# geoeo/ORB_SLAM3_V1.0

Hardware: AMD Instinct MI355X
Metric: frames/sec ORB extract+match, 752x480 8-level 1000-feat; bit-exact kp/desc (higher is better)
Workload: dtype u8

## Files before the change

### orb_slam3_v1.0_amd/csrc/fast_common.h

```cpp
#pragma once
#include <hip/hip_runtime.h>
#include <stdint.h>

namespace orbfe {

constexpr int kFastTW = 64, kFastTH = 32;

__device__ __forceinline__ bool arc9(uint32_t m)
{
    uint32_t m2 = m | (m << 16);
    uint32_t r = m2 & (m2 >> 1);
    r &= r >> 2;
    r &= r >> 4;
    r &= m2 >> 8;
    return (r & 0xffffu) != 0;
}

__device__ __forceinline__ bool corner_at_global(const uint8_t* __restrict__ img, int pitch, int x, int y, int th)
{
    const int8_t dy[16] = {3, 3, 2, 1, 0, -1, -2, -3, -3, -3, -2, -1, 0, 1, 2, 3};
    const int8_t dx[16] = {0, 1, 2, 3, 3, 3, 2, 1, 0, -1, -2, -3, -3, -3, -2, -1};
    const int v = img[(size_t)y * pitch + x];
    uint32_t mb = 0, md = 0;
#pragma unroll
    for (int k = 0; k < 16; k++) {
        const int d = (int)img[(size_t)(y + dy[k]) * pitch + x + dx[k]] - v;
        mb |= (uint32_t)(d > th) << k;
        md |= (uint32_t)(d < -th) << k;
    }
    return arc9(mb) || arc9(md);
}

}
```

### orb_slam3_v1.0_amd/csrc/kernels_fast.hip

```cpp
#include <cstdlib>

#include "launch.h"
#include "device_math.h"
#include "fast_common.h"

namespace orbfe {

constexpr int kImgW = kFastTW + 8, kImgH = kFastTH + 8;
constexpr int kScH = kFastTH + 2;
constexpr int kScW = kFastTW + 2;
constexpr int kScPitch = kImgW;
constexpr int kScoreOfs = 3 * kImgW + 3;
constexpr int kMaxTileCand = (kFastTW / 2) * (kFastTH / 2);
constexpr int kTmpH = kFastTH + 4;
constexpr int kQCap = 2304;
static_assert(kQCap >= kScH * kScW && kQCap % 2 == 0, "stage A geometry");

typedef unsigned short u16x2 __attribute__((ext_vector_type(2)));


__device__ __forceinline__ unsigned long long mask_le_u32(uint32_t x, uint32_t bound)
{
    unsigned long long m;
    asm("v_cmp_le_u32_e64 %0, %1, %2" : "=s"(m) : "v"(x), "s"(bound));
// ... 32 lines not shown
{
    unsigned long long m;
    if (vbound) asm("v_cmp_lt_i32_e64 %0, %1, %2" : "=s"(m) : "v"(a), "v"(b));
    else asm("v_cmp_lt_i32_e64 %0, %1, %2" : "=s"(m) : "v"(a), "s"(b));
    return m;
}
__device__ __forceinline__ void masked_lds_write_b8(unsigned long long mask, uint32_t addr, uint32_t v)
{
    unsigned long long save;
    asm volatile("s_and_saveexec_b64 %0, %1\n\tds_write_b8 %2, %3\n\ts_mov_b64 exec, %0" : "=&s"(save) : "s"(mask), "v"(addr), "v"(v) : "scc", "memory");
}
__device__ __forceinline__ void masked_lds_write_b16(unsigned long long mask, uint32_t addr, uint32_t v)
{
    unsigned long long save;
    asm volatile("s_and_saveexec_b64 %0, %1\n\tds_write_b16 %2, %3\n\ts_mov_b64 exec, %0" : "=&s"(save) : "s"(mask), "v"(addr), "v"(v) : "scc", "memory");
}
__device__ __forceinline__ void lds_add(uint32_t* addr, uint32_t v)
{
    asm volatile("ds_add_u32 %0, %1" : : "v"((uint32_t)(uintptr_t)addr), "v"(v) : "memory");
}

__device__ __forceinline__ uint32_t lds_add_rtn(uint32_t* addr, uint32_t v)
{
    uint32_t old;
    asm volatile("ds_add_rtn_u32 %0, %1, %2\n\ts_waitcnt lgkmcnt(0)" : "=&v"(old) : "v"((uint32_t)(uintptr_t)addr), "v"(v) : "memory");
    return old;
}

__device__ __forceinline__ uint32_t min16(uint32_t a, uint32_t b)
{
    uint32_t r;
    asm("v_min_u16 %0, %1, %2" : "=v"(r) : "v"(a), "v"(b));
    return r;
}
__device__ __forceinline__ uint32_t max16(uint32_t a, uint32_t b)
{
    uint32_t r;
    asm("v_max_u16 %0, %1, %2" : "=v"(r) : "v"(a), "v"(b));
    return r;
}
__device__ __forceinline__ uint32_t sub16(uint32_t a, uint32_t b)
{
    uint32_t r;
    asm("v_sub_u16 %0, %1, %2" : "=v"(r) : "v"(a), "v"(b));
    return r;
}
__device__ __forceinline__ uint32_t maxi16(uint32_t a, uint32_t b)
{
    uint32_t r;
    asm("v_max_i16 %0, %1, %2" : "=v"(r) : "v"(a), "v"(b));
    return r;
}

__device__ __forceinline__ uint32_t arc_max_of_min(const uint32_t (&p)[16])
{
    uint32_t S[16], Pf[16];
    S[7] = p[7];
    S[15] = p[15];
#pragma unroll
    for (int k = 6; k >= 0; k--) {
        S[k] = min16(p[k], S[k + 1]);
        S[k + 8] = min16(p[k + 8], S[k + 9]);
    }
    Pf[0] = p[0];
    Pf[8] = p[8];
#pragma unroll
    for (int k = 1; k < 7; k++) {
        Pf[k] = min16(p[k], Pf[k - 1]);
        Pf[k + 8] = min16(p[k + 8], Pf[k + 7]);
    }
    Pf[7] = S[0];
    Pf[15] = S[8];
    uint32_t a[16];
#pragma unroll
    for (int k = 0; k < 8; k++) {
        a[k] = min16(S[k], Pf[k + 8]);
        a[k + 8] = min16(S[k + 8], Pf[k]);
    }
#pragma unroll
    for (int st = 8; st >= 1; st >>= 1)
#pragma unroll
        for (int k = 0; k < st; k++) a[k] = max16(a[k], a[k + st]);
    return a[0];
}

__device__ __forceinline__ uint32_t arc_min_of_max(const uint32_t (&p)[16])
{
    uint32_t S[16], Pf[16];
    S[7] = p[7];
    S[15] = p[15];
#pragma unroll
    for (int k = 6; k >= 0; k--) {
        S[k] = max16(p[k], S[k + 1]);
        S[k + 8] = max16(p[k + 8], S[k + 9]);
    }
    Pf[0] = p[0];
    Pf[8] = p[8];
#pragma unroll
    for (int k = 1; k < 7; k++) {
        Pf[k] = max16(p[k], Pf[k - 1]);
        Pf[k + 8] = max16(p[k + 8], Pf[k + 7]);
    }
    Pf[7] = S[0];
    Pf[15] = S[8];
    uint32_t a[16];
#pragma unroll
    for (int k = 0; k < 8; k++) {
        a[k] = max16(S[k], Pf[k + 8]);
        a[k + 8] = max16(S[k + 8], Pf[k]);
    }
#pragma unroll
    for (int st = 8; st >= 1; st >>= 1)
#pragma unroll
        for (int k = 0; k < st; k++) a[k] = min16(a[k], a[k + st]);
    return a[0];
}

__device__ __forceinline__ unsigned long long mask_th_i16(int th, uint32_t m)
{
    unsigned long long r;
    asm("v_cmp_lt_i16_e64 %0, %1, %2" : "=s"(r) : "s"(th), "v"(m));
    return r;
}

__device__ __forceinline__ int queue_slot1(uint32_t m, int th, unsigned long long mask, uint32_t entry, int stepV, int qNext)
{
    unsigned long long save;
    uint32_t tmp;
    int cnt;
    asm volatile("v_cmp_lt_i16_e32 vcc, %8, %3\n\t"
                 "s_and_b64 vcc, vcc, %4\n\t"
                 "s_and_saveexec_b64 %0, vcc\n\t"
                 "v_mbcnt_lo_u32_b32 %1, vcc_lo, 0\n\t"
                 "v_mbcnt_hi_u32_b32 %1, vcc_hi, %1\n\t"
                 "v_mad_i32_i24 %1, %1, %6, %7\n\t"
                 "ds_write_b16 %1, %5\n\t"
                 "s_mov_b64 exec, %0\n\t"
                 "s_bcnt1_i32_b64 %2, vcc"
                 : "=&s"(save), "=&v"(tmp), "=s"(cnt)
                 : "v"(m), "s"(mask), "v"(entry), "v"(stepV), "s"(qNext), "s"(th)
                 : "vcc", "scc", "memory");
    return cnt;
}

template <int MODE>
__global__ __launch_bounds__(256) void fast_blur_kernel(const PipelineDesc* __restrict__ P,
                                                        const uint32_t* __restrict__ tileInfo,
                                                        const uint8_t* __restrict__ gray0, size_t gray0FrameStride,
                                                        int gray0Pitch, int gray0Aligned4,
                                                        uint8_t* __restrict__ ws, uint32_t* __restrict__ cand,
                                                        uint32_t* __restrict__ counters,
                                                        uint16_t* __restrict__ tileRows)
{
    __shared__ uint32_t sRow[kFastTH];
    __shared__ __attribute__((aligned(16))) uint8_t sImg[kImgH + 1][kImgW];
    __shared__ __attribute__((aligned(16))) uint32_t sTmp[kTmpH / 2][kFastTW];
    __shared__ __attribute__((aligned(16))) uint8_t sScore[kScH + 1][kScPitch];
    __shared__ uint32_t sCand[kMaxTileCand];
    __shared__ uint32_t sCnt[4];
    __shared__ uint32_t sBase;
    __shared__ __attribute__((aligned(4))) uint16_t sQA[kQCap];
    static_assert(sizeof(uint16_t) * kScH * kScW <= sizeof(uint32_t) * (kTmpH / 2) * kFastTW, "corner queue must fit the blur buffer");
    uint16_t* const sQB = reinterpret_cast<uint16_t*>(&sTmp[0][0]);
    __shared__ uint32_t sQ[3];

    const int f = blockIdx.x;
    const int tile = blockIdx.y;
    const int nL = P->nLevels;
    const uint32_t ti = tileInfo[tile];
    const int l = (int)(ti >> 24);
    const LevelDesc& L = P->lv[l];
    const int w = L.w, h = L.h;
    const int x0 = (int)(ti & 0xfffu) * kFastTW;
    const int y0 = (int)((ti >> 12) & 0xfffu) * kFastTH;
    const int minTh = P->minTh, iniTh = P->iniTh;

    const uint8_t* src;
    int spitch;
    bool aligned;
    if (l == 0) {
        src = gray0 + (size_t)f * gray0FrameStride;
        spitch = gray0Pitch;
        aligned = gray0Aligned4 != 0;
    } else {
        src = ws + L.imgOff + (size_t)f * L.imgFrameStride;
        spitch = L.pitch;
        aligned = true;
    }

    const int tid = threadIdx.x;
    const int lane = tid & 63;
    if (tid < 4) sCnt[tid] = 0;
    if (tid < 3) sQ[tid] = 0;
    if (tid < kFastTH) sRow[tid] = 0;

    if (aligned) {
        if (tid < 14 * (kImgW / 4)) {
            const int r0 = tid / (kImgW / 4);
            const int c4 = tid - r0 * (kImgW / 4);
            const int gx = x0 - 4 + 4 * c4;
            const bool colIn = gx >= 0 && gx < w;
            uint32_t wv[3];
            if (y0 >= 4 && y0 + kFastTH + 4 <= h) {
                uint32_t off = __umul24((unsigned)(y0 - 4 + r0), (unsigned)spitch) + (unsigned)gx;
                const uint32_t step = 14u * (unsigned)spitch;
#pragma unroll
                for (int k = 0; k < 3; k++) {
                    wv[k] = 0;
                    if (colIn && r0 + 14 * k < kImgH) wv[k] = *reinterpret_cast<const uint32_t*>(src + off);
                    off += step;
                }
            } else {
#pragma unroll
                for (int k = 0; k < 3; k++) {
                    const int r = r0 + 14 * k;
                    wv[k] = 0;
                    if (colIn && r < kImgH)
                        wv[k] = *reinterpret_cast<const uint32_t*>(src + (size_t)reflect_near(y0 - 4 + r, h) * spitch + gx);
                }
            }
#pragma unroll
            for (int k = 0; k < 3; k++) {
                const int r = r0 + 14 * k;
                if (colIn && r < kImgH) *reinterpret_cast<uint32_t*>(&sImg[r][4 * c4]) = wv[k];
            }
        }
        const int cR = w - x0 + 4;
        const bool patchL = x0 == 0, patchR = cR + 1 < kImgW;
        if (patchL || patchR) {
            __syncthreads();
            if (tid < kImgH) {
                if (patchL) {
                    sImg[tid][2] = sImg[tid][6];
                    sImg[tid][3] = sImg[tid][5];
                }
            } else if (tid >= 64 && tid < 64 + kImgH) {
                if (patchR) {
                    sImg[tid - 64][cR] = sImg[tid - 64][cR - 2];
                    sImg[tid - 64][cR + 1] = sImg[tid - 64][cR - 3];
                }
            }
        }
    } else {
        for (int e = tid; e < kImgH * (kImgW / 4); e += 256) {
            const int r = e / (kImgW / 4);
            const int c4 = e - r * (kImgW / 4);
            const uint8_t* row = src + (size_t)reflect_near(y0 - 4 + r, h) * spitch;
            uint32_t wv = 0;
#pragma unroll
            for (int i = 0; i < 4; i++) wv |= (uint32_t)row[reflect_near(x0 - 4 + 4 * c4 + i, w)] << (8 * i);
            *reinterpret_cast<uint32_t*>(&sImg[r][4 * c4]) = wv;
        }
    }
    __syncthreads();

    if constexpr ((MODE & 1) != 0) {
    for (int e = tid; e < (kTmpH / 2) * (kFastTW / 4); e += 256) {
        const int j = e / (kFastTW / 4);
        const int xl = (e - j * (kFastTW / 4)) * 4;
        uint32_t o[2][4];
#pragma unroll
        for (int half = 0; half < 2; half++) {
            const uint32_t* rowp = reinterpret_cast<const uint32_t*>(&sImg[2 * j + half + 2][xl]);
            const uint32_t w0 = rowp[0], w1 = rowp[1], w2 = rowp[2];
            uint32_t win[5];
            win[0] = __builtin_amdgcn_alignbyte(w1, w0, 2);
            win[1] = __builtin_amdgcn_alignbyte(w1, w0, 3);
            win[2] = w1;
            win[3] = __builtin_amdgcn_alignbyte(w2, w1, 1);
            win[4] = __builtin_amdgcn_alignbyte(w2, w1, 2);
#pragma unroll
            for (int i = 0; i < 4; i++)
                o[half][i] = __builtin_amdgcn_udot4(win[i + 1], 0x16000000u,
                                                    __builtin_amdgcn_udot4(win[i], 0x3E583E16u, 0u, false), false);
        }
        uint4 pk;
        pk.x = o[0][0] | (o[1][0] << 16);
        pk.y = o[0][1] | (o[1][1] << 16);
        pk.z = o[0][2] | (o[1][2] << 16);
        pk.w = o[0][3] | (o[1][3] << 16);
        *reinterpret_cast<uint4*>(&sTmp[j][xl]) = pk;
    }
    __syncthreads();
    }

    const int wv = __builtin_amdgcn_readfirstlane(tid >> 6);
    if (wv >= 2) {
        if constexpr ((MODE & 2) != 0)
            for (int e = tid - 128; e < (kScH + 1) * (kScPitch / 4); e += 128) reinterpret_cast<uint32_t*>(&sScore[0][0])[e] = 0;
        if constexpr ((MODE & 1) != 0) {
            uint8_t* dst = ws + L.blurOff + (size_t)f * L.blurFrameStride;
            const int dpitch = L.pitch;
            const int xl = (tid & 15) * 4;
#pragma unroll 1
            for (int yp = (tid - 128) >> 4; yp < kFastTH / 2; yp += 8) {
                const int gy = y0 + 2 * yp, gx = x0 + xl;
                if (gy < h && gx < w) {
                    const uint4 p0 = *reinterpret_cast<const uint4*>(&sTmp[yp][xl]);
                    const uint4 p1 = *reinterpret_cast<const uint4*>(&sTmp[yp + 1][xl]);
                    const uint4 p2 = *reinterpret_cast<const uint4*>(&sTmp[yp + 2][xl]);
                    const uint32_t c0[4] = {p0.x, p0.y, p0.z, p0.w}, c1[4] = {p1.x, p1.y, p1.z, p1.w}, c2[4] = {p2.x, p2.y, p2.z, p2.w};
                    uint32_t ev[4], od[4];
#pragma unroll
                    for (int i = 0; i < 4; i++) {
                        const u16x2 a = __builtin_bit_cast(u16x2, c0[i]), b = __builtin_bit_cast(u16x2, c1[i]), c = __builtin_bit_cast(u16x2, c2[i]);
                        uint32_t acc = __builtin_amdgcn_udot2(a, __builtin_bit_cast(u16x2, 0x003E0016u), 32768u, false);
                        acc = __builtin_amdgcn_udot2(b, __builtin_bit_cast(u16x2, 0x003E0058u), acc, false);
                        ev[i] = __builtin_amdgcn_udot2(c, __builtin_bit_cast(u16x2, 0x00000016u), acc, false);
                        acc = __builtin_amdgcn_udot2(a, __builtin_bit_cast(u16x2, 0x00160000u), 32768u, false);
                        acc = __builtin_amdgcn_udot2(b, __builtin_bit_cast(u16x2, 0x0058003Eu), acc, false);
                        od[i] = __builtin_amdgcn_udot2(c, __builtin_bit_cast(u16x2, 0x0016003Eu), acc, false);
                    }
                    const uint32_t outE = __builtin_amdgcn_perm(ev[1], ev[0], 0x0c0c0602u) |
                                          (__builtin_amdgcn_perm(ev[3], ev[2], 0x0c0c0602u) << 16);
                    const uint32_t outO = __builtin_amdgcn_perm(od[1], od[0], 0x0c0c0602u) |
                                          (__builtin_amdgcn_perm(od[3], od[2], 0x0c0c0602u) << 16);
                    uint8_t* drow = dst + (size_t)gy * dpitch;
                    const bool odd = gy + 1 < h;
                    if (gx + 3 < w) {
                        *reinterpret_cast<uint32_t*>(drow + gx) = outE;
                        if (odd) *reinterpret_cast<uint32_t*>(drow + dpitch + gx) = outO;
                    } else {
                        for (int i = 0; gx + i < w; i++) {
                            drow[gx + i] = (uint8_t)(outE >> (8 * i));
                            if (odd) drow[dpitch + gx + i] = (uint8_t)(outO >> (8 * i));
                        }
                    }
// ... 156 lines not shown
            masked_lds_add(mPre, rowLds + 4u * oy, select_by_mask(mHi, 0x10001u, 1u));
            if (mKeep) {
                uint32_t wbase = 0;
                if (lane == 0) wbase = lds_add_rtn(&sCnt[0], (uint32_t)__popcll(mKeep));
                wbase = __builtin_amdgcn_readfirstlane(wbase);
                const uint32_t rank = __builtin_amdgcn_mbcnt_hi((uint32_t)(mKeep >> 32), __builtin_amdgcn_mbcnt_lo((uint32_t)mKeep, 0u));
                masked_lds_write_b32(mKeep, candLds + 4u * (wbase + rank), pack_cand(x0 + (int)ox, y0 + (int)oy, (int)sc));
            }
        }
        if (lane == 0) {
            if (nPreW) lds_add(&sCnt[2], nPreW);
            if (nPreHiW) lds_add(&sCnt[3], nPreHiW);
            if (nKeepHiW) lds_add(&sCnt[1], nKeepHiW);
        }
        asm volatile("s_waitcnt lgkmcnt(0)" ::: "memory");
    }
    __syncthreads();

    }

    if (tid < kFastTH) {
        const uint32_t v = sRow[tid];
        tileRows[((size_t)f * P->totalTiles + tile) * kFastTH + tid] = (uint16_t)((v & 0xffu) | ((v >> 16) << 8));
    }

    uint32_t* cnt = counters + ((size_t)f * nL + l) * kCntWords;
    const uint32_t nTile = sCnt[0];
    if (tid == 0) {
        uint32_t base = 0;
        if constexpr ((MODE & 256) != 0) base = (uint32_t)tile * 8u;
        else if (nTile) base = atomicAdd(&cnt[kCntCand], nTile);
        if (sCnt[1]) atomicAdd(&cnt[kCntHigh], sCnt[1]);
        if (sCnt[2]) atomicAdd(&cnt[kCntPreLow], sCnt[2]);
        if (sCnt[3]) atomicAdd(&cnt[kCntPreHigh], sCnt[3]);
        sBase = base;
    }
    __syncthreads();
    if (nTile) {
        const uint32_t base = sBase;
        uint32_t* out = cand + L.candOff + (size_t)f * L.candCap;
        for (uint32_t i = tid; i < nTile; i += 256) {
            if (base + i < (uint32_t)L.candCap) out[base + i] = sCand[i];
            else atomicOr(&cnt[kCntStatus], (uint32_t)kFlagCandOverflow);
        }
    }
}

void fast_tiles_for(int w, int h, int* tx, int* ty)
{
    *tx = (w + kFastTW - 1) / kFastTW;
    *ty = (h + kFastTH - 1) / kFastTH;
}

uint32_t fast_tile_info(int level, int tileX, int tileY) { return ((uint32_t)level << 24) | ((uint32_t)tileY << 12) | (uint32_t)tileX; }

void launch_fast_blur(hipStream_t s, int frames, int totalTiles, const PipelineDesc* dP, const uint32_t* dTileInfo,
                      const uint8_t* gray0, size_t gray0FrameStride, int gray0Pitch, int gray0Aligned4, uint8_t* ws,
                      uint32_t* cand, uint32_t* counters, uint16_t* tileRows)
{
    dim3 block(256);
    dim3 grid(frames, totalTiles);
#define ORBFE_LAUNCH_FB(M)                                                                                          \
    hipLaunchKernelGGL(fast_blur_kernel<M>, grid, block, 0, s, dP, dTileInfo, gray0, gray0FrameStride, gray0Pitch, \
                       gray0Aligned4, ws, cand, counters, tileRows)
#ifdef ORBFE_ABLATION
    static const int mode = [] {
        const char* e = getenv("ORBFE_FAST_MODE");
        return e ? atoi(e) & 1023 : 3;
    }();
    switch (mode) {
    case 0: ORBFE_LAUNCH_FB(0); break;
    case 1: ORBFE_LAUNCH_FB(1); break;
    case 2: ORBFE_LAUNCH_FB(2); break;
    case 6: ORBFE_LAUNCH_FB(6); break;
    case 10: ORBFE_LAUNCH_FB(10); break;
    case 26: ORBFE_LAUNCH_FB(26); break;
    case 67: ORBFE_LAUNCH_FB(67); break;
    case 195: ORBFE_LAUNCH_FB(195); break;
    case 259: ORBFE_LAUNCH_FB(259); break;
    case 515: ORBFE_LAUNCH_FB(515); break;
    case 42: ORBFE_LAUNCH_FB(42); break;
    default: ORBFE_LAUNCH_FB(3); break;
    }
#else
    ORBFE_LAUNCH_FB(3);
#endif
#undef ORBFE_LAUNCH_FB
}

}
```

### orb_slam3_v1.0_amd/csrc/launch.h

```cpp
#pragma once
#include "orbfe_internal.h"

namespace orbfe {

void launch_resize(hipStream_t s, int frames, const uint8_t* src, size_t srcFrameStride, int sw, int sh,
                   int spitch, int srcAligned4, uint8_t* dst, size_t dstFrameStride, int dw, int dh, int dpitch,
                   const uint32_t* xtab, const uint32_t* ytab);

bool pyramid_level_fits(const uint32_t* xtab, const uint32_t* ytab, int sw, int sh, int dw, int dh);
void launch_pyramid_level(hipStream_t s, int frames, const PipelineDesc* dP, int level, int dw, int dh, const uint8_t* gray0,
                          size_t gray0FrameStride, int gray0Pitch, uint8_t* ws, const uint32_t* tabs);

void launch_pyramid_chain(hipStream_t s, int frames, const PipelineDesc* dP, const PipelineDesc& hostP, int l0, int depth,
                          const uint8_t* gray0, size_t gray0FrameStride, int gray0Pitch, uint8_t* ws, const uint32_t* tabs,
                          uint32_t* zero = nullptr, int nZeroPerFrame = 0);

void fast_tiles_for(int w, int h, int* tx, int* ty);
uint32_t fast_tile_info(int level, int tileX, int tileY);
void launch_fast_blur(hipStream_t s, int frames, int totalTiles, const PipelineDesc* dP, const uint32_t* dTileInfo,
                      const uint8_t* gray0, size_t gray0FrameStride, int gray0Pitch, int gray0Aligned4, uint8_t* ws,
                      uint32_t* cand, uint32_t* counters, uint16_t* tileRows);

int quadtree_node_capacity(int maxNodeCap);
size_t quadtree_scratch_bytes_per_block(int maxNodeCap);
void launch_quadtree(hipStream_t s, int frames, int nLevels, int maxNodeCap, const PipelineDesc* dP,
                     const uint32_t* cand, uint16_t* nodeOf, uint32_t* counters, uint32_t* lvlKp,
                     const uint8_t* gray0, size_t gray0FrameStride, int gray0Pitch, const uint8_t* ws,
                     const uint16_t* tileRows, uint8_t* scratch);

void launch_orient_brief(hipStream_t s, int frames, int kpCapFrame, const PipelineDesc* dP, const uint8_t* gray0,
                         size_t gray0FrameStride, int gray0Pitch, const uint8_t* ws, const uint32_t* counters,
                         const uint32_t* lvlKp, orbfe_keypoint* kpOut, uint8_t* descOut, int* nOut,
                         int* perLevelOut, int* statusOut, const int* kpBase, int nLevels);

void launch_clock_probe(hipStream_t s, unsigned long long* dOut2, unsigned ticks);

}
```

### orb_slam3_v1.0_amd/csrc/orbfe_host.cpp

```cpp
#include <atomic>
#include <cmath>
#include <cstdio>
#include <cstdlib>
#include <cstring>
#include <map>
#include <mutex>
#include <new>
#include <condition_variable>
#include <functional>
#include <string>
#include <thread>
#include <vector>

#include "launch.h"
#include "match.h"
#include "match_common.h"
#include "match_proj.h"
#include "keyframe.h"
#include "prep.h"
#include "vocab.h"

using namespace orbfe;

namespace {

constexpr int kEventSets = 128;

size_t align_up(size_t v, size_t a) { return (v + a - 1) / a * a; }

const char* kStageNames[ORBFE_NUM_STAGES] = {"pyramid_resize", "fast_nms_blur",
                                             "quadtree", "orient_brief", "total"};

}

struct orbfe_map;
struct orbfe_stream;

struct orbfe_handle {
    orbfe_params prm{};
    int device = 0;
    int nLevels = 0;
    double scaleFactorD = 0.0;
    float sf[kMaxLevels]{}, inv[kMaxLevels]{}, sig2[kMaxLevels]{}, invSig2[kMaxLevels]{};
    PipelineDesc P{};
    PipelineDesc* dP = nullptr;
    int maxBatch = 1;
    int maxNodeCap = 0;

    uint8_t* ws = nullptr;
    size_t wsBytes = 0;
    uint32_t* dCand = nullptr;
    uint16_t* dNodeOf = nullptr;
    size_t candWordsPerBatch = 0;
    uint32_t* dCounters = nullptr;
    uint32_t* dLvlKp = nullptr;
    uint16_t* dTileRows = nullptr;
    uint8_t* dQtScratch = nullptr;
    uint32_t* dTabs = nullptr;
    uint32_t* dTileInfo = nullptr;
    bool pyrFits[kMaxLevels]{};
    float* dSf = nullptr;

    uint8_t* dIn = nullptr;
    int dInPitch = 0;
    uint8_t* hIn = nullptr;
    uint8_t* dOutBlock = nullptr;
    uint8_t* hOutBlock = nullptr;
    size_t outBlockBytes = 0, offStatus = 0, offPer = 0, offKp = 0, offDesc = 0;
    orbfe_keypoint* dKp = nullptr;
    uint8_t* dDesc = nullptr;
    int* dN = nullptr;
    int* dStatus = nullptr;
    int* dPer = nullptr;
    orbfe_keypoint* hKp = nullptr;
    uint8_t* hDesc = nullptr;
    int* hN = nullptr;
    int* hStatus = nullptr;
    int* hPer = nullptr;
    std::map<int, hipGraphExec_t> graphs;
    bool useGraph = true;
    int graphCaptures = 0, captureFailures = 0;
    int captureFailStreak = 0;

    hipStream_t stream = nullptr;
    bool timing = false;
    hipEvent_t ev[kEventSets][ORBFE_NUM_STAGES]{};
    int evHead = 0, evCount = 0;

    const uint8_t* lastGray = nullptr;
    size_t lastStride = 0;
    int lastPitch = 0, lastBatch = 0;

    MatchScratch match;

    struct TrackKey {
        int Mb, inPitch, gridCols, gridRows, farPoints;
        float minX, minY, invW, invH, th, nnRatio, thFar;
        const void* map;
    };
    struct TrackGraph {
        TrackKey key;
        hipGraphExec_t exec;
    };
    MatchScratch trackMatch;
    uint8_t* dTrkIn = nullptr;
    uint8_t* hTrkIn = nullptr;
    uint8_t* dTrkOut = nullptr;
    uint8_t* hTrkOut = nullptr;
    int trkCapM = 0;
    std::vector<TrackGraph> trackGraphs;
    struct RefKey {
        int inPitch, levelsup, checkOri;
        float nnRatio;
// ... 215 lines not shown
        fpl[nL - 1] = std::max(p->n_features - sum, 0);
    }

    PipelineDesc& P = h->P;
    memset(&P, 0, sizeof P);
    P.nLevels = nL;
    P.nFast = p->n_fast_features;
    P.iniTh = p->ini_th_fast;
    P.minTh = p->min_th_fast;
    size_t wsOff = 0, candOff = 0, tabOff = 0;
    int tileBase = 0, kpBase = 0;
    const size_t B = (size_t)p->max_batch;
    int status = ORBFE_OK;
    for (int l = 0; l < nL; l++) {
        LevelDesc& L = P.lv[l];
        if (l == 0) {
            L.w = p->image_width;
            L.h = p->image_height;
        } else {
            L.w = cv_round_f(h->inv[l] * (float)p->image_width);
            L.h = cv_round_f(h->inv[l] * (float)p->image_height);
        }
        if (L.w < 16 || L.h < 16) { status = ORBFE_ERR_UNSUPPORTED; break; }
        L.pitch = (int)align_up((size_t)L.w, kPitchAlign);
        L.nFeatures = fpl[l];
        L.nIni = (int)roundf((float)L.w / (float)L.h);
        if (L.nIni < 1) { status = ORBFE_ERR_UNSUPPORTED; break; }
        L.hX = (float)L.w / (float)L.nIni;
        L.nodeCap = std::max(L.nFeatures + 3, 4 * L.nIni);
        L.candCap = ((L.w + 1) / 2) * ((L.h + 1) / 2);
        fast_tiles_for(L.w, L.h, &L.tilesX, &L.tilesY);
        L.tileBase = tileBase;
        tileBase += L.tilesX * L.tilesY;
        L.kpBase = kpBase;
        kpBase += L.nodeCap;
        L.invScale = h->inv[l];
        L.scaledPatch = (int)(kPatch * h->inv[l]);
        const size_t frameBytes = align_up((size_t)L.pitch * L.h, 256);
        L.imgFrameStride = frameBytes;
        L.blurFrameStride = frameBytes;
        if (l > 0) {
            L.imgOff = wsOff;
            wsOff += frameBytes * B;
        }
        L.blurOff = wsOff;
        wsOff += frameBytes * B;
        L.candOff = candOff;
        candOff += (size_t)L.candCap * B;
        tabOff = align_up(tabOff, 4);
        L.xtabOff = tabOff;
        tabOff += align_up((size_t)L.w, 4);
        L.ytabOff = tabOff;
        tabOff += align_up((size_t)L.h, 4);
        h->maxNodeCap = std::max(h->maxNodeCap, L.nodeCap);
    }
    if (status == ORBFE_OK && quadtree_node_capacity(h->maxNodeCap) == 0) status = ORBFE_ERR_UNSUPPORTED;
    if (status != ORBFE_OK) {
        delete h;
        return status;
    }
    P.kpCapFrame = kpBase;
    P.totalTiles = tileBase;
    for (int l = 0; l < 8; l++) P.tileBaseTab[l] = l < nL ? P.lv[l].tileBase : 0x7fffffff;
    h->wsBytes = wsOff;
    h->candWordsPerBatch = candOff;

    std::vector<uint32_t> tabs(tabOff ? tabOff : 1, 0);
    for (int l = 1; l < nL; l++) {
        fill_resize_table(tabs, P.lv[l].xtabOff, P.lv[l - 1].w, P.lv[l].w);
        fill_resize_table(tabs, P.lv[l].ytabOff, P.lv[l - 1].h, P.lv[l].h);
    }

    for (int l = 1; l < nL; l++)
        if (pyramid_level_fits(tabs.data() + P.lv[l].xtabOff, tabs.data() + P.lv[l].ytabOff, P.lv[l - 1].w, P.lv[l - 1].h, P.lv[l].w,
                               P.lv[l].h))
            h->pyrFits[l] = true;

#define CREATE_CHK(call)                                                  \
    do {                                                                  \
        hipError_t e_ = (call);                                           \
        if (e_ != hipSuccess) {                                           \
            int rc_ = e_ == hipErrorOutOfMemory ? ORBFE_ERR_OUT_OF_MEMORY : ORBFE_ERR_HIP; \
            destroy_impl(h);                                              \
            return rc_;                                                   \
        }                                                                 \
    } while (0)

    CREATE_CHK(hipStreamCreateWithFlags(&h->stream, hipStreamNonBlocking));
    CREATE_CHK(hipMalloc(&h->dP, sizeof(PipelineDesc)));
    CREATE_CHK(hipMalloc(&h->ws, h->wsBytes + 256));
    CREATE_CHK(hipMalloc(&h->dCand, candOff * sizeof(uint32_t)));
    CREATE_CHK(hipMalloc(&h->dNodeOf, candOff * sizeof(uint16_t)));
    CREATE_CHK(hipMalloc(&h->dCounters, B * nL * kCntWords * sizeof(uint32_t)));
    CREATE_CHK(hipMalloc(&h->dLvlKp, B * (size_t)P.kpCapFrame * sizeof(uint32_t)));
    CREATE_CHK(hipMalloc(&h->dTileRows, B * (size_t)P.totalTiles * 32 * sizeof(uint16_t)));
    if (quadtree_scratch_bytes_per_block(h->maxNodeCap))
        CREATE_CHK(hipMalloc(&h->dQtScratch, quadtree_scratch_bytes_per_block(h->maxNodeCap) * B * nL));
    CREATE_CHK(hipMalloc(&h->dTabs, tabs.size() * sizeof(uint32_t)));
    {
        std::vector<uint32_t> info((size_t)P.totalTiles);
        for (int l = 0; l < nL; l++)
            for (int ty = 0; ty < P.lv[l].tilesY; ty++)
                for (int tx = 0; tx < P.lv[l].tilesX; tx++) info[P.lv[l].tileBase + ty * P.lv[l].tilesX + tx] = fast_tile_info(l, tx, ty);
        CREATE_CHK(hipMalloc(&h->dTileInfo, info.size() * sizeof(uint32_t)));
        CREATE_CHK(copy_sync(h->dTileInfo, info.data(), info.size() * sizeof(uint32_t), hipMemcpyHostToDevice, h->stream));
    }
    CREATE_CHK(hipMalloc(&h->dSf, kMaxLevels * sizeof(float)));
    CREATE_CHK(copy_sync(h->dSf, h->sf, kMaxLevels * sizeof(float), hipMemcpyHostToDevice, h->stream));
    CREATE_CHK(copy_sync(h->dP, &P, sizeof P, hipMemcpyHostToDevice, h->stream));
    CREATE_CHK(copy_sync(h->dTabs, tabs.data(), tabs.size() * sizeof(uint32_t), hipMemcpyHostToDevice, h->stream));

    h->dInPitch = (int)align_up((size_t)p->image_width, kPitchAlign);
    const size_t inFrame = (size_t)h->dInPitch * p->image_height;
    const size_t cap = (size_t)P.kpCapFrame;
    CREATE_CHK(hipMalloc(&h->dIn, inFrame * B));
    CREATE_CHK(hipHostMalloc(&h->hIn, inFrame * B));
    {
        size_t off = 0;
        auto take = [&](size_t bytes) { const size_t o = off; off = align_up(off + bytes, 256); return o; };
        take(B * sizeof(int));
        h->offStatus = take(B * sizeof(int));
        h->offPer = take(B * nL * sizeof(int));
        h->offKp = take(B * cap * sizeof(orbfe_keypoint));
        h->offDesc = take(B * cap * ORBFE_DESC_BYTES);
        h->outBlockBytes = off;
    }
    CREATE_CHK(hipMalloc(&h->dOutBlock, h->outBlockBytes));
    CREATE_CHK(hipHostMalloc(&h->hOutBlock, h->outBlockBytes));
    h->dN = reinterpret_cast<int*>(h->dOutBlock);
    h->dStatus = reinterpret_cast<int*>(h->dOutBlock + h->offStatus);
    h->dPer = reinterpret_cast<int*>(h->dOutBlock + h->offPer);
    h->dKp = reinterpret_cast<orbfe_keypoint*>(h->dOutBlock + h->offKp);
    h->dDesc = h->dOutBlock + h->offDesc;
    h->hN = reinterpret_cast<int*>(h->hOutBlock);
    h->hStatus = reinterpret_cast<int*>(h->hOutBlock + h->offStatus);
    h->hPer = reinterpret_cast<int*>(h->hOutBlock + h->offPer);
    h->hKp = reinterpret_cast<orbfe_keypoint*>(h->hOutBlock + h->offKp);
    h->hDesc = h->hOutBlock + h->offDesc;
#ifdef ORBFE_DIAG
    h->useGraph = getenv("ORBFE_NO_GRAPH") == nullptr;
#endif
    CREATE_CHK(hipEventCreateWithFlags(&h->evExtract, hipEventDisableTiming));
    CREATE_CHK(hipEventCreateWithFlags(&h->evMatch, hipEventDisableTiming));
    h->match.busy = h->evMatch;
    for (auto& set : h->ev)
        for (auto& e : set) CREATE_CHK(hipEventCreate(&e));
#undef CREATE_CHK
    *out = h;
    return ORBFE_OK;
}

void orbfe_destroy(orbfe_handle* h) { destroy_impl(h); }

int orbfe_get_levels(const orbfe_handle* h) { return h ? h->nLevels : 0; }
float orbfe_get_scale_factor(const orbfe_handle* h) { return h ? (float)h->scaleFactorD : 0.f; }

int orbfe_get_scale_tables(const orbfe_handle* h, float* sf, float* inv, float* s2, float* is2)
{
    if (!h) return ORBFE_ERR_INVALID_ARG;
    for (int i = 0; i < h->nLevels; i++) {
        if (sf) sf[i] = h->sf[i];
        if (inv) inv[i] = h->inv[i];
        if (s2) s2[i] = h->sig2[i];
        if (is2) is2[i] = h->invSig2[i];
    }
    return ORBFE_OK;
}

int orbfe_get_level_info(const orbfe_handle* h, int* fpl, int* lw, int* lh)
{
    if (!h) return ORBFE_ERR_INVALID_ARG;
    for (int i = 0; i < h->nLevels; i++) {
        if (fpl) fpl[i] = h->P.lv[i].nFeatures;
        if (lw) lw[i] = h->P.lv[i].w;
        if (lh) lh[i] = h->P.lv[i].h;
    }
    return ORBFE_OK;
}

int orbfe_max_keypoints(const orbfe_handle* h) { return h ? h->P.kpCapFrame : 0; }

int orbfe_set_stage_timing(orbfe_handle* h, int enabled)
{
    if (!h) return ORBFE_ERR_INVALID_ARG;
    h->timing = enabled != 0;
    h->evHead = h->evCount = 0;
    return ORBFE_OK;
}

int orbfe_get_stage_ms(orbfe_handle* h, float ms[ORBFE_NUM_STAGES], int* n_calls)
{
    if (!h || !ms || !n_calls) return ORBFE_ERR_INVALID_ARG;
    HIPCHK(h, hipSetDevice(h->device));
// ... 5 lines not shown
        for (int s = 0; s + 1 < ORBFE_NUM_STAGES; s++) {
            float t = 0.f;
            HIPCHK(h, hipEventElapsedTime(&t, e[s], e[s + 1]));
            ms[s] += t;
        }
        float t = 0.f;
        HIPCHK(h, hipEventElapsedTime(&t, e[0], e[ORBFE_NUM_STAGES - 1]));
        ms[ORBFE_NUM_STAGES - 1] += t;
    }
    *n_calls = n;
    return ORBFE_OK;
}

static int extract_chain(orbfe_handle* h, const uint8_t* d_gray, size_t frame_stride, int pitch, int batch,
                         orbfe_keypoint* d_kp, uint8_t* d_desc, int* d_n, int* d_per, int* d_status, void* stream_);

int orbfe_extract_batch_device(orbfe_handle* h, const uint8_t* d_gray, size_t frame_stride, int pitch,
                               int batch, orbfe_keypoint* d_kp, uint8_t* d_desc, int* d_n, int* d_per,
                               void* stream_)
{
    if (!h) return ORBFE_ERR_INVALID_ARG;
    std::lock_guard<std::mutex> lk(h->mu);
    return extract_chain(h, d_gray, frame_stride, pitch, batch, d_kp, d_desc, d_n, d_per, nullptr, stream_);
}

}

static int extract_chain(orbfe_handle* h, const uint8_t* d_gray, size_t frame_stride, int pitch, int batch,
                         orbfe_keypoint* d_kp, uint8_t* d_desc, int* d_n, int* d_per, int* d_status, void* stream_)
{
    if (!h || !d_gray || !d_kp || !d_desc || !d_n) return ORBFE_ERR_INVALID_ARG;
    if (batch < 1 || batch > h->maxBatch || pitch < h->prm.image_width || pitch >= (1 << 24)) return ORBFE_ERR_INVALID_ARG;
    const int aligned4 = ((reinterpret_cast<uintptr_t>(d_gray) | (uintptr_t)pitch | (uintptr_t)frame_stride) & 3u) == 0;
    const size_t rowEnd = aligned4 ? (size_t)((h->prm.image_width + 3) & ~3) : (size_t)h->prm.image_width;
    if (batch > 1 && frame_stride < (size_t)pitch * (h->prm.image_height - 1) + rowEnd) return ORBFE_ERR_INVALID_ARG;
    if ((size_t)pitch * (h->prm.image_height - 1) + (size_t)((h->prm.image_width + 3) & ~3) >= (size_t)0x7ffffff0u)
        return ORBFE_ERR_INVALID_ARG;
    HIPCHK(h, hipSetDevice(h->device));
    hipStream_t s = stream_ ? (hipStream_t)stream_ : h->stream;
    hipStreamCaptureStatus capturing = hipStreamCaptureStatusNone;
    if (hipStreamIsCapturing(s, &capturing) != hipSuccess) (void)hipGetLastError();
    if (capturing == hipStreamCaptureStatusNone) {
        const int rc = scratch_acquire(h, h->extractUsed, h->extractStream, h->evExtract, s);
        if (rc != ORBFE_OK) return rc;
    }
    const PipelineDesc& P = h->P;
    const int nL = P.nLevels;
    hipEvent_t* ev = nullptr;
    if (h->timing) {
        ev = h->ev[h->evHead];
        h->evHead = (h->evHead + 1) % kEventSets;
        h->evCount++;
    }
    const bool chainPyr = (long long)batch * nL <= 64 && !ev && nL > 1;
    if (!chainPyr) HIPCHK(h, hipMemsetAsync(h->dCounters, 0, (size_t)batch * nL * kCntWords * sizeof(uint32_t), s));
    if (ev) HIPCHK(h, hipEventRecord(ev[0], s));
    for (int l = 1; chainPyr && l < nL;) {
        const int left = nL - l;
        const int depth = left >= 5 ? 2 : std::min(left, 3);
        launch_pyramid_chain(s, batch, h->dP, P, l - 1, depth, d_gray, frame_stride, pitch, h->ws, h->dTabs,
                             l == 1 ? h->dCounters : nullptr, nL * kCntWords);
        l += depth;
    }
    for (int l = chainPyr ? nL : 1; l < nL; l++) {
        const LevelDesc& S = P.lv[l - 1];
        const LevelDesc& D = P.lv[l];
        if (h->pyrFits[l] && (l > 1 || aligned4)) {
            launch_pyramid_level(s, batch, h->dP, l, D.w, D.h, d_gray, frame_stride, pitch, h->ws, h->dTabs);
            continue;
        }
        const uint8_t* src = l == 1 ? d_gray : h->ws + S.imgOff;
        const size_t sstride = l == 1 ? frame_stride : S.imgFrameStride;
        const int spitch = l == 1 ? pitch : S.pitch;
        launch_resize(s, batch, src, sstride, S.w, S.h, spitch, l == 1 ? aligned4 : 1, h->ws + D.imgOff, D.imgFrameStride, D.w, D.h,
                      D.pitch, h->dTabs + D.xtabOff, h->dTabs + D.ytabOff);
    }
    if (ev) HIPCHK(h, hipEventRecord(ev[1], s));
    launch_fast_blur(s, batch, P.totalTiles, h->dP, h->dTileInfo, d_gray, frame_stride, pitch, aligned4, h->ws, h->dCand, h->dCounters,
                     h->dTileRows);
    if (ev) HIPCHK(h, hipEventRecord(ev[2], s));
    launch_quadtree(s, batch, nL, h->maxNodeCap, h->dP, h->dCand, h->dNodeOf, h->dCounters, h->dLvlKp, d_gray, frame_stride,
                    pitch, h->ws, h->dTileRows, h->dQtScratch);
    if (ev) HIPCHK(h, hipEventRecord(ev[3], s));
    int kpBase[kMaxLevels];
    for (int l = 0; l < nL; l++) kpBase[l] = P.lv[l].kpBase;
    launch_orient_brief(s, batch, P.kpCapFrame, h->dP, d_gray, frame_stride, pitch, h->ws, h->dCounters, h->dLvlKp,
                        d_kp, d_desc, d_n, d_per, d_status, kpBase, nL);
    if (ev) HIPCHK(h, hipEventRecord(ev[4], s));
    HIPCHK(h, hipGetLastError());
    h->lastGray = d_gray;
    h->lastStride = frame_stride;
    h->lastPitch = pitch;
    h->lastBatch = batch;
    if (capturing == hipStreamCaptureStatusNone) return extract_scratch_release(h, s);
    return ORBFE_OK;
}

extern "C" {

static int check_device_flags(orbfe_handle* h, int batch)
{
    for (int b = 0; b < batch; b++)
        if (h->hStatus[b]) {
            char buf[128];
            snprintf(buf, sizeof buf, "device guard flags 0x%x at frame %d", (unsigned)h->hStatus[b], b);
            h->err = buf;
            return ORBFE_ERR_INTERNAL;
        }
    return ORBFE_OK;
}

static int extract_host_enqueue(orbfe_handle* h, int batch, int inPitch, hipStream_t s)
{
    const int nL = h->nLevels;
    const size_t inFrame = (size_t)h->dInPitch * h->prm.image_height;
    const size_t cap = (size_t)h->P.kpCapFrame;
    const int rc = extract_chain(h, h->dIn, inFrame, inPitch, batch, h->dKp, h->dDesc, h->dN, h->dPer, h->dStatus, s);
    if (rc != ORBFE_OK) return rc;
    if (batch == h->maxBatch) {
        HIPCHK(h, hipMemcpyAsync(h->hOutBlock, h->dOutBlock, h->outBlockBytes, hipMemcpyDeviceToHost, s));
    } else {
        HIPCHK(h, hipMemcpyAsync(h->hN, h->dN, batch * sizeof(int), hipMemcpyDeviceToHost, s));
        HIPCHK(h, hipMemcpyAsync(h->hStatus, h->dStatus, batch * sizeof(int), hipMemcpyDeviceToHost, s));
        HIPCHK(h, hipMemcpyAsync(h->hPer, h->dPer, (size_t)batch * nL * sizeof(int), hipMemcpyDeviceToHost, s));
        HIPCHK(h, hipMemcpyAsync(h->hKp, h->dKp, batch * cap * sizeof(orbfe_keypoint), hipMemcpyDeviceToHost, s));
        HIPCHK(h, hipMemcpyAsync(h->hDesc, h->dDesc, batch * cap * ORBFE_DESC_BYTES, hipMemcpyDeviceToHost, s));
    }
    return ORBFE_OK;
}

struct CaptureStream {
    hipStream_t s = nullptr;
// ... 2398 lines not shown
```

### orb_slam3_v1.0_amd/csrc/orbfe_internal.h

```cpp
#pragma once

#include <hip/hip_runtime.h>
#include <stdint.h>

#include "../../include/orbfe.h"

inline hipError_t copy_sync(void* dst, const void* src, size_t bytes, hipMemcpyKind kind, hipStream_t s)
{
    if (bytes == 0) return hipSuccess;
    const hipError_t e = hipMemcpyAsync(dst, src, bytes, kind, s);
    return e != hipSuccess ? e : hipStreamSynchronize(s);
}
inline hipError_t memset_sync(void* dst, int value, size_t bytes, hipStream_t s)
{
    if (bytes == 0) return hipSuccess;
    const hipError_t e = hipMemsetAsync(dst, value, bytes, s);
    return e != hipSuccess ? e : hipStreamSynchronize(s);
}

int orbfe_stream_create_copy_threads(orbfe_handle* h, int slots, int slot_frames, int copy_threads, orbfe_stream** out);
void orbfe_stream_release_track(orbfe_stream* st);
void orbfe_stream_drain(orbfe_stream* st);

namespace orbfe {

constexpr int kMaxLevels = ORBFE_MAX_LEVELS;
constexpr int kEdge = 5;
constexpr int kHalfPatch = 15;
constexpr int kPatch = 31;
constexpr int kPitchAlign = 64;

constexpr int kCoordBits = 12;
constexpr uint32_t kCoordMask = (1u << kCoordBits) - 1;
__host__ __device__ inline uint32_t pack_cand(int x, int y, int score)
{
    return ((uint32_t)score << 24) | ((uint32_t)y << kCoordBits) | (uint32_t)x;
}
__host__ __device__ inline int cand_x(uint32_t c) { return (int)(c & kCoordMask); }
__host__ __device__ inline int cand_y(uint32_t c) { return (int)((c >> kCoordBits) & kCoordMask); }
__host__ __device__ inline int cand_score(uint32_t c) { return (int)(c >> 24); }
__host__ __device__ inline uint32_t cand_key(uint32_t c) { return c & 0x00FFFFFFu; }

enum Counter {
    kCntCand = 0,
    kCntHigh = 1,
    kCntPreLow = 2,
    kCntPreHigh = 3,
    kCntKp = 4,
    kCntStatus = 5,
    kCntWords = 8
};

enum DeviceFlag : uint32_t {
    kFlagNodeOverflow = 1u,
    kFlagRoundLimit = 2u,
    kFlagCandOverflow = 4u,
};

struct LevelDesc {
    int w, h, pitch;
    int nFeatures;
    int nIni;
    float hX;
    int nodeCap;
    int candCap;
    int tilesX, tilesY;
    int tileBase;
    int kpBase;
    float invScale;
    int scaledPatch;
    uint32_t pad_;
    size_t imgOff;
    size_t imgFrameStride;
    size_t blurOff, blurFrameStride;
    size_t candOff;
    size_t xtabOff, ytabOff;
};

struct PipelineDesc {
    int nLevels;
    int nFast;
    int iniTh, minTh;
    int kpCapFrame;
    int totalTiles;
    int tileBaseTab[8];
    LevelDesc lv[kMaxLevels];
};

}
```

Before: 219,800.

## Add optional fused pyramid build in FAST kernel and slim arc/blur arithmetic

Adds an optional path where each FAST tile kernel also bilinearly resamples the next pyramid level from its shared-memory tile, launched level by level. The path is off by default, gated by a frame threshold constant set to zero and an env override. It also replaces the prefix/suffix min-max network for the FAST score with a shorter pairwise arc reduction. The blur's alignbyte windowing is replaced by udot4 calls with pre-shifted weight constants. The smaller arithmetic changes aim to cut VALU work in the FAST/blur kernel. The fused path trades extra launches for skipping separate pyramid kernels.

```diff
diff --git a/orb_slam3_v1.0_amd/csrc/fast_common.h b/orb_slam3_v1.0_amd/csrc/fast_common.h
--- a/orb_slam3_v1.0_amd/csrc/fast_common.h
+++ b/orb_slam3_v1.0_amd/csrc/fast_common.h
@@ -5,6 +5,8 @@
 namespace orbfe {
 
 constexpr int kFastTW = 64, kFastTH = 32;
+
+constexpr int kFusedPyramidMinFrames = 0;
 
 __device__ __forceinline__ bool arc9(uint32_t m)
 {
diff --git a/orb_slam3_v1.0_amd/csrc/kernels_fast.hip b/orb_slam3_v1.0_amd/csrc/kernels_fast.hip
--- a/orb_slam3_v1.0_amd/csrc/kernels_fast.hip
+++ b/orb_slam3_v1.0_amd/csrc/kernels_fast.hip
@@ -108,69 +108,29 @@
     return r;
 }
 
-__device__ __forceinline__ uint32_t arc_max_of_min(const uint32_t (&p)[16])
-{
-    uint32_t S[16], Pf[16];
-    S[7] = p[7];
-    S[15] = p[15];
-#pragma unroll
-    for (int k = 6; k >= 0; k--) {
-        S[k] = min16(p[k], S[k + 1]);
-        S[k + 8] = min16(p[k + 8], S[k + 9]);
-    }
-    Pf[0] = p[0];
-    Pf[8] = p[8];
-#pragma unroll
-    for (int k = 1; k < 7; k++) {
-        Pf[k] = min16(p[k], Pf[k - 1]);
-        Pf[k + 8] = min16(p[k + 8], Pf[k + 7]);
-    }
-    Pf[7] = S[0];
-    Pf[15] = S[8];
-    uint32_t a[16];
-#pragma unroll
-    for (int k = 0; k < 8; k++) {
-        a[k] = min16(S[k], Pf[k + 8]);
-        a[k + 8] = min16(S[k + 8], Pf[k]);
-    }
-#pragma unroll
-    for (int st = 8; st >= 1; st >>= 1)
-#pragma unroll
-        for (int k = 0; k < st; k++) a[k] = max16(a[k], a[k + st]);
+template <bool DARK>
+__device__ __forceinline__ uint32_t arc_extreme(const uint32_t (&p)[16])
+{
+    auto lo = [](uint32_t a, uint32_t b) { return DARK ? max16(a, b) : min16(a, b); };
+    auto hi = [](uint32_t a, uint32_t b) { return DARK ? min16(a, b) : max16(a, b); };
+    uint32_t m2[8], m4[8], a[8];
+#pragma unroll
+    for (int j = 0; j < 8; j++) m2[j] = lo(p[2 * j + 1], p[(2 * j + 2) & 15]);
+#pragma unroll
+    for (int j = 0; j < 8; j++) m4[j] = lo(m2[j], m2[(j + 1) & 7]);
+#pragma unroll
+    for (int j = 0; j < 8; j++) {
+        const uint32_t core = lo(m4[j], m4[(j + 2) & 7]);
+        a[j] = lo(core, hi(p[2 * j], p[(2 * j + 9) & 15]));
+    }
+#pragma unroll
+    for (int st = 4; st >= 1; st >>= 1)
+#pragma unroll
+        for (int k = 0; k < st; k++) a[k] = hi(a[k], a[k + st]);
     return a[0];
 }
-
-__device__ __forceinline__ uint32_t arc_min_of_max(const uint32_t (&p)[16])
-{
-    uint32_t S[16], Pf[16];
-    S[7] = p[7];
-    S[15] = p[15];
-#pragma unroll
-    for (int k = 6; k >= 0; k--) {
-        S[k] = max16(p[k], S[k + 1]);
-        S[k + 8] = max16(p[k + 8], S[k + 9]);
-    }
-    Pf[0] = p[0];
-    Pf[8] = p[8];
-#pragma unroll
-    for (int k = 1; k < 7; k++) {
-        Pf[k] = max16(p[k], Pf[k - 1]);
-        Pf[k + 8] = max16(p[k + 8], Pf[k + 7]);
-    }
-    Pf[7] = S[0];
-    Pf[15] = S[8];
-    uint32_t a[16];
-#pragma unroll
-    for (int k = 0; k < 8; k++) {
-        a[k] = max16(S[k], Pf[k + 8]);
-        a[k + 8] = max16(S[k + 8], Pf[k]);
-    }
-#pragma unroll
-    for (int st = 8; st >= 1; st >>= 1)
-#pragma unroll
-        for (int k = 0; k < st; k++) a[k] = min16(a[k], a[k + st]);
-    return a[0];
-}
+__device__ __forceinline__ uint32_t arc_max_of_min(const uint32_t (&p)[16]) { return arc_extreme<false>(p); }
+__device__ __forceinline__ uint32_t arc_min_of_max(const uint32_t (&p)[16]) { return arc_extreme<true>(p); }
 
 __device__ __forceinline__ unsigned long long mask_th_i16(int th, uint32_t m)
 {
@@ -199,9 +159,10 @@
     return cnt;
 }
 
-template <int MODE>
+template <int MODE, bool BUILD>
 __global__ __launch_bounds__(256) void fast_blur_kernel(const PipelineDesc* __restrict__ P,
-                                                        const uint32_t* __restrict__ tileInfo,
+                                                        const uint32_t* __restrict__ tileInfo, int tileBase,
+                                                        const uint32_t* __restrict__ tabs,
                                                         const uint8_t* __restrict__ gray0, size_t gray0FrameStride,
                                                         int gray0Pitch, int gray0Aligned4,
                                                         uint8_t* __restrict__ ws, uint32_t* __restrict__ cand,
@@ -221,7 +182,7 @@
     __shared__ uint32_t sQ[3];
 
     const int f = blockIdx.x;
-    const int tile = blockIdx.y;
+    const int tile = (int)blockIdx.y + tileBase;
     const int nL = P->nLevels;
     const uint32_t ti = tileInfo[tile];
     const int l = (int)(ti >> 24);
@@ -249,6 +210,20 @@
     if (tid < 4) sCnt[tid] = 0;
     if (tid < 3) sQ[tid] = 0;
     if (tid < kFastTH) sRow[tid] = 0;
+
+    int bXa = 0, bNX = 0, bYa = 0, bNY = 0;
+    uint32_t bXt = 0, bYt = 0;
+    if constexpr (BUILD) {
+        const uint32_t* own = tabs + L.ownOff;
+        const int tX = (int)(ti & 0xfffu), tY = (int)((ti >> 12) & 0xfffu);
+        bXa = (int)own[tX];
+        bNX = (int)own[tX + 1] - bXa;
+        bYa = (int)own[L.tilesX + 1 + tY];
+        bNY = (int)own[L.tilesX + 2 + tY] - bYa;
+        const LevelDesc& D = P->lv[l + 1];
+        if (lane < bNX) bXt = tabs[D.xtabOff + (size_t)(bXa + lane)];
+        if (lane < bNY) bYt = tabs[D.ytabOff + (size_t)(bYa + lane)];
+    }
 
     if (aligned) {
         if (tid < 14 * (kImgW / 4)) {
@@ -310,6 +285,31 @@
     }
     __syncthreads();
 
+    if constexpr (BUILD) {
+        static_assert(kFastTH == 32, "eight owned rows per wave at most");
+        const LevelDesc& D = P->lv[l + 1];
+        if (lane < bNX && bNY > 0) {
+            const uint32_t wx = bXt >> 16, wxc = 2048u - wx;
+            const uint8_t* sp = &sImg[0][0] + ((int)(bXt & 0xffffu) - (x0 - 4));
+            uint8_t* dcol = ws + D.imgOff + (size_t)f * D.imgFrameStride + (uint32_t)(bYa * D.pitch + bXa + lane);
+            const int q = __builtin_amdgcn_readfirstlane(tid >> 6);
+            uint32_t top[8], bot[8], wy[8];
+#pragma unroll
+            for (int k = 0; k < 8; k++) {
+                const uint32_t yt = (uint32_t)__builtin_amdgcn_readlane((int)bYt, min(q + 4 * k, bNY - 1));
+                const uint8_t* pr = sp + ((int)(yt & 0xffffu) - (y0 - 4)) * kImgW;
+                wy[k] = yt >> 16;
+                top[k] = __umul24(pr[0], wxc) + __umul24(pr[1], wx);
+                bot[k] = __umul24(pr[kImgW], wxc) + __umul24(pr[kImgW + 1], wx);
+            }
+#pragma unroll
+            for (int k = 0; k < 8; k++) {
+                const uint32_t v = __umul24(top[k], 2048u - wy[k]) + __umul24(bot[k], wy[k]) + (1u << 21);
+                if (q + 4 * k < bNY) dcol[(uint32_t)((q + 4 * k) * D.pitch)] = (uint8_t)(v >> 22);
+            }
+        }
+    }
+
     if constexpr ((MODE & 1) != 0) {
     for (int e = tid; e < (kTmpH / 2) * (kFastTW / 4); e += 256) {
         const int j = e / (kFastTW / 4);
@@ -319,16 +319,10 @@
         for (int half = 0; half < 2; half++) {
             const uint32_t* rowp = reinterpret_cast<const uint32_t*>(&sImg[2 * j + half + 2][xl]);
             const uint32_t w0 = rowp[0], w1 = rowp[1], w2 = rowp[2];
-            uint32_t win[5];
-            win[0] = __builtin_amdgcn_alignbyte(w1, w0, 2);
-            win[1] = __builtin_amdgcn_alignbyte(w1, w0, 3);
-            win[2] = w1;
-            win[3] = __builtin_amdgcn_alignbyte(w2, w1, 1);
-            win[4] = __builtin_amdgcn_alignbyte(w2, w1, 2);
-#pragma unroll
-            for (int i = 0; i < 4; i++)
-                o[half][i] = __builtin_amdgcn_udot4(win[i + 1], 0x16000000u,
-                                                    __builtin_amdgcn_udot4(win[i], 0x3E583E16u, 0u, false), false);
+            o[half][0] = __builtin_amdgcn_udot4(w1, 0x00163E58u, __builtin_amdgcn_udot4(w0, 0x3E160000u, 0u, false), false);
+            o[half][1] = __builtin_amdgcn_udot4(w1, 0x163E583Eu, __builtin_amdgcn_udot4(w0, 0x16000000u, 0u, false), false);
+            o[half][2] = __builtin_amdgcn_udot4(w2, 0x00000016u, __builtin_amdgcn_udot4(w1, 0x3E583E16u, 0u, false), false);
+            o[half][3] = __builtin_amdgcn_udot4(w2, 0x0000163Eu, __builtin_amdgcn_udot4(w1, 0x583E1600u, 0u, false), false);
         }
         uint4 pk;
         pk.x = o[0][0] | (o[1][0] << 16);
@@ -591,17 +585,42 @@
     *ty = (h + kFastTH - 1) / kFastTH;
 }
 
+bool fast_next_level_fits(const uint32_t* xtab, const uint32_t* ytab, int sw, int sh, int dw, int dh, uint32_t* own)
+{
+    int tx, ty;
+    fast_tiles_for(sw, sh, &tx, &ty);
+    bool ok = true;
+    auto fill = [&](const uint32_t* tab, int srcN, int dstN, int tile, int nTiles, uint32_t* o) {
+        int p = 0;
+        for (int t = 0; t <= nTiles; t++) {
+            while (p < dstN && (int)(tab[p] & 0xffffu) < t * tile) p++;
+            o[t] = (uint32_t)(t == nTiles ? dstN : p);
+            if (t > 0 && o[t] - o[t - 1] > 64u) ok = false;
+        }
+        for (int i = 0; i < dstN; i++)
+            if ((int)(tab[i] & 0xffffu) + 1 > srcN - 1 || (i > 0 && (tab[i] & 0xffffu) < (tab[i - 1] & 0xffffu))) ok = false;
+    };
+    fill(xtab, sw, dw, kFastTW, tx, own);
+    fill(ytab, sh, dh, kFastTH, ty, own + tx + 1);
+    return ok;
+}
+
 uint32_t fast_tile_info(int level, int tileX, int tileY) { return ((uint32_t)level << 24) | ((uint32_t)tileY << 12) | (uint32_t)tileX; }
 
-void launch_fast_blur(hipStream_t s, int frames, int totalTiles, const PipelineDesc* dP, const uint32_t* dTileInfo,
-                      const uint8_t* gray0, size_t gray0FrameStride, int gray0Pitch, int gray0Aligned4, uint8_t* ws,
-                      uint32_t* cand, uint32_t* counters, uint16_t* tileRows)
+void launch_fast_blur(hipStream_t s, int frames, int tileBase, int nTiles, bool buildNext, const PipelineDesc* dP,
+                      const uint32_t* dTileInfo, const uint32_t* dTabs, const uint8_t* gray0, size_t gray0FrameStride, int gray0Pitch,
+                      int gray0Aligned4, uint8_t* ws, uint32_t* cand, uint32_t* counters, uint16_t* tileRows)
 {
     dim3 block(256);
-    dim3 grid(frames, totalTiles);
-#define ORBFE_LAUNCH_FB(M)                                                                                          \
-    hipLaunchKernelGGL(fast_blur_kernel<M>, grid, block, 0, s, dP, dTileInfo, gray0, gray0FrameStride, gray0Pitch, \
-                       gray0Aligned4, ws, cand, counters, tileRows)
+    dim3 grid(frames, nTiles);
+    if (buildNext) {
+        hipLaunchKernelGGL((fast_blur_kernel<3, true>), grid, block, 0, s, dP, dTileInfo, tileBase, dTabs, gray0, gray0FrameStride,
+                           gray0Pitch, gray0Aligned4, ws, cand, counters, tileRows);
+        return;
+    }
+#define ORBFE_LAUNCH_FB(M)                                                                                                      \
+    hipLaunchKernelGGL((fast_blur_kernel<M, false>), grid, block, 0, s, dP, dTileInfo, tileBase, dTabs, gray0, gray0FrameStride, \
+                       gray0Pitch, gray0Aligned4, ws, cand, counters, tileRows)
 #ifdef ORBFE_ABLATION
     static const int mode = [] {
         const char* e = getenv("ORBFE_FAST_MODE");
diff --git a/orb_slam3_v1.0_amd/csrc/launch.h b/orb_slam3_v1.0_amd/csrc/launch.h
--- a/orb_slam3_v1.0_amd/csrc/launch.h
+++ b/orb_slam3_v1.0_amd/csrc/launch.h
@@ -17,9 +17,10 @@
 
 void fast_tiles_for(int w, int h, int* tx, int* ty);
 uint32_t fast_tile_info(int level, int tileX, int tileY);
-void launch_fast_blur(hipStream_t s, int frames, int totalTiles, const PipelineDesc* dP, const uint32_t* dTileInfo,
-                      const uint8_t* gray0, size_t gray0FrameStride, int gray0Pitch, int gray0Aligned4, uint8_t* ws,
-                      uint32_t* cand, uint32_t* counters, uint16_t* tileRows);
+void launch_fast_blur(hipStream_t s, int frames, int tileBase, int nTiles, bool buildNext, const PipelineDesc* dP,
+                      const uint32_t* dTileInfo, const uint32_t* dTabs, const uint8_t* gray0, size_t gray0FrameStride, int gray0Pitch,
+                      int gray0Aligned4, uint8_t* ws, uint32_t* cand, uint32_t* counters, uint16_t* tileRows);
+bool fast_next_level_fits(const uint32_t* xtab, const uint32_t* ytab, int sw, int sh, int dw, int dh, uint32_t* own);
 
 int quadtree_node_capacity(int maxNodeCap);
 size_t quadtree_scratch_bytes_per_block(int maxNodeCap);
diff --git a/orb_slam3_v1.0_amd/csrc/orbfe_host.cpp b/orb_slam3_v1.0_amd/csrc/orbfe_host.cpp
--- a/orb_slam3_v1.0_amd/csrc/orbfe_host.cpp
+++ b/orb_slam3_v1.0_amd/csrc/orbfe_host.cpp
@@ -13,6 +13,7 @@
 #include <vector>
 
 #include "launch.h"
+#include "fast_common.h"
 #include "match.h"
 #include "match_common.h"
 #include "match_proj.h"
@@ -59,6 +60,9 @@
     uint32_t* dTabs = nullptr;
     uint32_t* dTileInfo = nullptr;
     bool pyrFits[kMaxLevels]{};
+    bool fusedFits[kMaxLevels]{};
+    int fusedMinFrames = kFusedPyramidMinFrames;
+    bool fusedSplitOnly = false;
     float* dSf = nullptr;
 
     uint8_t* dIn = nullptr;
@@ -380,6 +384,9 @@
         tabOff += align_up((size_t)L.w, 4);
         L.ytabOff = tabOff;
         tabOff += align_up((size_t)L.h, 4);
+        tabOff = align_up(tabOff, 4);
+        L.ownOff = (uint32_t)tabOff;
+        tabOff += (size_t)L.tilesX + L.tilesY + 2;
         h->maxNodeCap = std::max(h->maxNodeCap, L.nodeCap);
     }
     if (status == ORBFE_OK && quadtree_node_capacity(h->maxNodeCap) == 0) status = ORBFE_ERR_UNSUPPORTED;
@@ -403,6 +410,9 @@
         if (pyramid_level_fits(tabs.data() + P.lv[l].xtabOff, tabs.data() + P.lv[l].ytabOff, P.lv[l - 1].w, P.lv[l - 1].h, P.lv[l].w,
                                P.lv[l].h))
             h->pyrFits[l] = true;
+    for (int l = 1; l < nL; l++)
+        h->fusedFits[l] = fast_next_level_fits(tabs.data() + P.lv[l].xtabOff, tabs.data() + P.lv[l].ytabOff, P.lv[l - 1].w, P.lv[l - 1].h,
+                                               P.lv[l].w, P.lv[l].h, tabs.data() + P.lv[l - 1].ownOff) && h->pyrFits[l];
 
 #define CREATE_CHK(call)                                                  \
     do {                                                                  \
@@ -467,6 +477,10 @@
     h->hDesc = h->hOutBlock + h->offDesc;
 #ifdef ORBFE_DIAG
     h->useGraph = getenv("ORBFE_NO_GRAPH") == nullptr;
+    if (const char* e = getenv("ORBFE_FUSED_PYRAMID")) {
+        h->fusedMinFrames = atoi(e) ? 1 : 0;
+        h->fusedSplitOnly = atoi(e) == 2;
+    }
 #endif
     CREATE_CHK(hipEventCreateWithFlags(&h->evExtract, hipEventDisableTiming));
     CREATE_CHK(hipEventCreateWithFlags(&h->evMatch, hipEventDisableTiming));
@@ -578,7 +592,8 @@
         h->evHead = (h->evHead + 1) % kEventSets;
         h->evCount++;
     }
-    const bool chainPyr = (long long)batch * nL <= 64 && !ev && nL > 1;
+    const bool fused = h->fusedMinFrames > 0 && batch >= h->fusedMinFrames && nL > 1;
+    const bool chainPyr = !fused && (long long)batch * nL <= 64 && !ev && nL > 1;
     if (!chainPyr) HIPCHK(h, hipMemsetAsync(h->dCounters, 0, (size_t)batch * nL * kCntWords * sizeof(uint32_t), s));
     if (ev) HIPCHK(h, hipEventRecord(ev[0], s));
     for (int l = 1; chainPyr && l < nL;) {
@@ -588,22 +603,32 @@
                              l == 1 ? h->dCounters : nullptr, nL * kCntWords);
         l += depth;
     }
-    for (int l = chainPyr ? nL : 1; l < nL; l++) {
+    auto pyramid_level = [&](int l) {
         const LevelDesc& S = P.lv[l - 1];
         const LevelDesc& D = P.lv[l];
         if (h->pyrFits[l] && (l > 1 || aligned4)) {
             launch_pyramid_level(s, batch, h->dP, l, D.w, D.h, d_gray, frame_stride, pitch, h->ws, h->dTabs);
-            continue;
+            return;
         }
         const uint8_t* src = l == 1 ? d_gray : h->ws + S.imgOff;
         const size_t sstride = l == 1 ? frame_stride : S.imgFrameStride;
         const int spitch = l == 1 ? pitch : S.pitch;
         launch_resize(s, batch, src, sstride, S.w, S.h, spitch, l == 1 ? aligned4 : 1, h->ws + D.imgOff, D.imgFrameStride, D.w, D.h,
                       D.pitch, h->dTabs + D.xtabOff, h->dTabs + D.ytabOff);
-    }
+    };
+    for (int l = chainPyr || (fused && !h->fusedSplitOnly) ? nL : 1; l < nL; l++) pyramid_level(l);
     if (ev) HIPCHK(h, hipEventRecord(ev[1], s));
-    launch_fast_blur(s, batch, P.totalTiles, h->dP, h->dTileInfo, d_gray, frame_stride, pitch, aligned4, h->ws, h->dCand, h->dCounters,
-                     h->dTileRows);
+    if (fused) {
+        for (int l = 0; l < nL; l++) {
+            const bool build = l + 1 < nL && h->fusedFits[l + 1] && !h->fusedSplitOnly;
+            launch_fast_blur(s, batch, P.lv[l].tileBase, P.lv[l].tilesX * P.lv[l].tilesY, build, h->dP, h->dTileInfo, h->dTabs, d_gray,
+                             frame_stride, pitch, aligned4, h->ws, h->dCand, h->dCounters, h->dTileRows);
+            if (l + 1 < nL && !build && !h->fusedSplitOnly) pyramid_level(l + 1);
+        }
+    } else {
+        launch_fast_blur(s, batch, 0, P.totalTiles, false, h->dP, h->dTileInfo, h->dTabs, d_gray, frame_stride, pitch, aligned4, h->ws,
+                         h->dCand, h->dCounters, h->dTileRows);
+    }
     if (ev) HIPCHK(h, hipEventRecord(ev[2], s));
     launch_quadtree(s, batch, nL, h->maxNodeCap, h->dP, h->dCand, h->dNodeOf, h->dCounters, h->dLvlKp, d_gray, frame_stride,
                     pitch, h->ws, h->dTileRows, h->dQtScratch);
diff --git a/orb_slam3_v1.0_amd/csrc/orbfe_internal.h b/orb_slam3_v1.0_amd/csrc/orbfe_internal.h
--- a/orb_slam3_v1.0_amd/csrc/orbfe_internal.h
+++ b/orb_slam3_v1.0_amd/csrc/orbfe_internal.h
@@ -69,7 +69,7 @@
     int kpBase;
     float invScale;
     int scaledPatch;
-    uint32_t pad_;
+    uint32_t ownOff;
     size_t imgOff;
     size_t imgFrameStride;
     size_t blurOff, blurFrameStride;
```

New measurement: 224,000 (median of 6 runs). 1.9% higher.
